# Zhouxunzhe/ManiSkill

Measured on AMD Instinct MI355X. Metric: env-steps/sec (whole node), PickCube-v1 state-obs 4096 envs/GPU, higher is better.
Workload: dtype f32; 1 GPU; PickCube-v1, Panda, state obs [N,42], pd_joint_delta_pos, num_envs=4096/GPU, sim 100 Hz / control 20 Hz = 5 substeps, 15+1 solver iterations, random actions 2*U-1, no resets inside the timed region; envs_per_gpu=4096, substeps=5, parallelism=env-sharded x1, no collective on the env path, solver_overflow_envs=0

## Files before the change

### __graft_entry__.py

```python
import os
import subprocess
import sys

ROOT = os.path.dirname(os.path.abspath(__file__))
if ROOT not in sys.path:
    sys.path.insert(0, ROOT)

HIPCC = os.environ.get("HIPCC", "/opt/rocm/bin/hipcc")
NATIVE_DIR = os.path.join(ROOT, "maniskill_amd", "_native")
SRC = os.path.join(ROOT, "maniskill_amd", "csrc", "mssim_kernels.hip")
LIB = os.path.join(NATIVE_DIR, "libmssim.so")


def _stale(target, sources):
    if not os.path.exists(target):
        return True
    t = os.path.getmtime(target)
    return any(os.path.getmtime(s) > t for s in sources)


def build(force: bool = False) -> None:
    os.makedirs(NATIVE_DIR, exist_ok=True)
    csrc = os.path.join(ROOT, "maniskill_amd", "csrc")
    deps = [os.path.join(csrc, f) for f in os.listdir(csrc)] + [os.path.join(ROOT, "include", h) for h in ("mssim.h", "mssim_hip_tasks.h")]
    if force or _stale(LIB, deps):
        tmp = f"{LIB}.{os.getpid()}.tmp"
        cmd = [HIPCC, "-O3", "--offload-arch=gfx950", "-std=c++17", "-shared", "-fPIC", "-Wno-unused-value", "-fno-hip-fp32-correctly-rounded-divide-sqrt", "-o", tmp, SRC]
        try:
            subprocess.run(cmd, check=True)
            os.replace(tmp, LIB)
        finally:
            if os.path.exists(tmp):
                os.remove(tmp)
    subprocess.run(["make", "-s", "-C", os.path.join(ROOT, "oracle")], check=True)
    import maniskill_amd
    from maniskill_amd import native

    native.NativeLib.load(LIB)


def smoke() -> None:
    import numpy as np
    import torch

    from maniskill_amd.model.scenes import panda_tabletop_model
    from maniskill_amd.physx.system import MssimSystem
    from tests import oracle_backend as ob

    assert torch.cuda.is_available(), "smoke() needs a GPU"
    build()
    model = panda_tabletop_model()
    N = 64
    g = torch.Generator().manual_seed(0)
    rest = torch.tensor([0, np.pi / 8, 0, -np.pi * 5 / 8, 0, np.pi * 3 / 4, np.pi / 4, 0.04, 0.04])
    q0 = rest + 0.02 * torch.randn(N, 9, generator=g)
    q0[:, 7:] = 0.04
    tq = q0.clone()
    tq[:, :7] += 0.1 * (2 * torch.rand(N, 7, generator=g) - 1)
    outs = []
    for dev, backend in (("cuda:0", None), ("cpu", "oracle")):
        if backend is None:
            px = MssimSystem(device=dev)
            px.gpu_init(model, N)
        else:
            px = ob.make_system(model, N, precision="f64")
        px.cuda_articulation_qpos.torch()[:] = q0.to(dev)
# ... 16 lines not shown
```

### include/mssim.h

```cpp
#ifndef MSSIM_H
#define MSSIM_H

#include <stdint.h>

#ifdef __cplusplus
extern "C" {
#endif

#define MSSIM_ABI_VERSION 6
#define MSSIM_MAX_ANGULAR_VELOCITY 100.0f
#define MSSIM_MAX_JOINT_VELOCITY 100.0f
#define MSSIM_MPR_TOLERANCE 1e-5f
#define MSSIM_PCM_SLOTS 16
#define MSSIM_PCM_DRIFT 5e-3f
#define MSSIM_PCM_MOVE 1e-3f
#define MSSIM_PCM_ROT_TRACE 2.9996f
#define MSSIM_PCM_TILT 0.05f
#define MSSIM_PCM_GROW 6
#define MSSIM_PCM_MERGE 2e-3f
#ifndef MSSIM_PGS_EXIT_TOLERANCE
#define MSSIM_PGS_EXIT_TOLERANCE 1e-6f
#endif
#define MSSIM_WAKE_TIME 0.4f
#define MSSIM_MAX_DOF 16
#define MSSIM_MAX_FREE 8
#define MSSIM_MAX_POINTS 4
#define MSSIM_MAX_HULL_VERTS 64
#define MSSIM_TRI_SLACK 4e-3f
#define MSSIM_TRI_TIE 1e-5f
#define MSSIM_MAX_TRI_HITS 32
#define MSSIM_MAX_TRI_TASKS 56
#define MSSIM_TRI_RANGE_STEPS 4
#define MSSIM_PATCH_COS 0.985f
#define MSSIM_PATCH_TIE_SEP 1e-5f
#define MSSIM_PATCH_SLACK 4e-3f
#define MSSIM_PATCH_TIE_REL 1e-3f
#define MSSIM_MAX_CONTACTS 52
#define MSSIM_MAX_HITS 64
#define MSSIM_MAX_RAW_POINTS 128

enum {
  MSSIM_OVERFLOW_HITS = 1,
  MSSIM_OVERFLOW_CONVEX = 2,
  MSSIM_OVERFLOW_RAW = 4,
  MSSIM_OVERFLOW_CONTACTS = 8,
  MSSIM_OVERFLOW_TRI = 16
};
enum { MSSIM_JOINT_REVOLUTE = 0, MSSIM_JOINT_PRISMATIC = 1 };
enum { MSSIM_DRIVE_FORCE = 0, MSSIM_DRIVE_ACCELERATION = 1 };
enum {
  MSSIM_SHAPE_PLANE = 0,
  MSSIM_SHAPE_BOX = 1,
// ... 200 lines not shown
```

### maniskill_amd/csrc/mssim_kernels.hip

```cpp
#include <hip/hip_runtime.h>

#include <cmath>
#include <cstdint>
#include <cstdio>
#include <cstdlib>
#include <cstring>
#include <algorithm>
#include <string>
#include <vector>

#include "../../include/mssim.h"
#include "../../include/mssim_hip_tasks.h"
#include "mssim_collide.h"

static_assert(sizeof(mssim_stack_task) <= sizeof(mssim_peg_task) && alignof(mssim_stack_task) <= alignof(mssim_peg_task), "tail_task union would grow");
static_assert(sizeof(mssim_pusht_task) <= sizeof(mssim_peg_task) && alignof(mssim_pusht_task) <= alignof(mssim_peg_task), "tail_task union would grow");

#define MAXC 52

struct DevModel {
  int n_dof, n_tendon, n_link, n_free, n_kin, n_shape, n_pair;
  const int *dof_parent, *dof_type, *body_gravity, *tendon_dof, *link_body, *free_gravity;
  const unsigned* dof_anc;
  const float *dof_frame, *dof_axis, *dof_limit, *dof_drive, *dof_armature, *body_inertial, *tendon_param, *link_frame;
  const float *free_inertial, *free_damping;
  const int *shape_type, *shape_kind, *shape_index, *shape_row, *shape_hull, *pair_shape;
  const int* pair_packed;
  const float *shape_frame, *shape_param, *shape_material, *shape_bound, *hull_verts;
  const float* shape_center;
  const float* dof_pack;
  const float* shape_pack;
  const float* shape_half;
  const float* tri_soup;
  const float* tri_bvh;
  const int* pair_mesh_slot;
  const int *shape_env_slot, *free_env_slot;
  const float *env_shape_frame, *env_shape_param, *env_shape_bound, *env_free_inertial;
  float gx, gy, gz, dt, contact_offset, rest_offset, erp, max_depen, sleep_threshold;
  int pos_iters, vel_iters;
};

struct DevState {
  int N;
  float *root, *q, *qd, *qt, *qdt, *qf, *qacc;
  float *free_s, *free_force, *kin;
  float* free_wake;
  float* pcm;
  int* pcm_tick;
  float* warm;
  float* tri_clear;
  float *bodypose, *bodyvel;
  float* bodyaux;
  int* pair_cnt;
  float* pair_imp;
  int* hit_list;
  float* rows;
  int* overflow;
  const float* act;
  int act_dim;
  const int* act_col;
  const float *act_lo, *act_hi;
  const int* act_flags;
  const float* act_qpos;
  float* act_target;
  float* act_target_vel;
  unsigned tail_fetch;
  mssim_buffers tail_buf;
  union { mssim_pick_task pick; mssim_push_task push; mssim_peg_task peg; mssim_stack_task stack; mssim_pusht_task pusht; } tail_task;
  const int* tail_pairs; int tail_npairs;
  float *tail_obs, *tail_reward, *tail_head;
  uint8_t* tail_flags;
};

struct TopoDyn {
  static constexpr int MAXD = MSSIM_MAX_DOF;
  static constexpr bool STATIC = false;
  static constexpr int UNROLL = 1;
  int nd;
  const int* par;
  const int* typ;
  const unsigned* ancm;
  MS_DEV TopoDyn(const DevModel& M) : nd(M.n_dof), par(M.dof_parent), typ(M.dof_type), ancm(M.dof_anc) {}
  MS_DEV int n() const { return nd; }
  MS_DEV int parent(int j) const { return par[j]; }
  MS_DEV bool revolute(int j) const { return typ[j] == MSSIM_JOINT_REVOLUTE; }
  MS_DEV unsigned anc(int j) const { return ancm[j]; }
};
struct TopoPanda {
  static constexpr int MAXD = 9;
  static constexpr bool STATIC = true;
// ... 745 lines not shown
  const int n = M.n_dof;
  const pose_t root = pose_soa(S.root, 0, N, e);
  const m3 Rr = qmat(root.q);
  const int b = M.link_body[link];
  const pose_t Pb = b < 0 ? root : pose_soa(S.bodypose, 7 * b, N, e);
  const f3 pe = pmul(Pb, pose_from(M.link_frame + 7 * link)).p;
  const unsigned path = b < 0 ? 0u : (M.dof_anc[b] | (1u << b));
  float* o = out + (size_t)e * 6 * n;
  for (int j = 0; j < n; j++) {
    f3 jv = f3{0, 0, 0}, jw = f3{0, 0, 0};
    if ((path >> j) & 1u) {
      const f3 a = f3{SOA(S.bodyaux, 6 * j), SOA(S.bodyaux, 6 * j + 1), SOA(S.bodyaux, 6 * j + 2)};
      const f3 an = f3{SOA(S.bodyaux, 6 * j + 3), SOA(S.bodyaux, 6 * j + 4), SOA(S.bodyaux, 6 * j + 5)};
      if (M.dof_type[j] == MSSIM_JOINT_REVOLUTE) { jv = cross(a, pe - an); jw = a; }
      else jv = a;
      jv = mtmulv(Rr, jv);
      jw = mtmulv(Rr, jw);
    }
    o[0 * n + j] = jv.x; o[1 * n + j] = jv.y; o[2 * n + j] = jv.z;
    o[3 * n + j] = jw.x; o[4 * n + j] = jw.y; o[5 * n + j] = jw.z;
  }
}

__global__ void k_fill(float* dst, float v, size_t count) {
  size_t i = blockIdx.x * (size_t)blockDim.x + threadIdx.x;
  if (i < count) dst[i] = v;
}
__global__ void k_i2f(const int* src, float* dst, size_t count) {
  size_t i = blockIdx.x * (size_t)blockDim.x + threadIdx.x;
  if (i < count) dst[i] = (float)src[i];
}

#include "mssim_solve16.h"

struct mssim_sim {
  int device = 0;
  int N = 0;
  DevModel M{};
  DevState S{};
  mssim_buffers buf{};
  std::vector<void*> allocs;
  std::vector<float> drive_host;
  float* d_drive = nullptr;
  bool panda = false;
  bool has_tri = false;
  int rows_per_env = 1;
  bool dirty = true;
  int n_cu = 256;
  unsigned deferred_fetch = 0u;
  const float* deferred_action = nullptr; int deferred_adim = 0, deferred_nsub = 0; hipStream_t deferred_stream = nullptr;
  std::vector<float> h_dof_pack; float* d_dof_pack = nullptr;
  std::vector<int32_t> h_shape_row, h_pair_shape;
  int* d_pick_pairs = nullptr; int n_pick_pairs = 0; int pick_rows[3] = {-1, -1, -1};
  long long n_tail_steps = 0;
  std::vector<int*> queries;
  std::vector<int> query_n;
  std::vector<int> query_kind;
  std::string err;
  int* d_act_col = nullptr; float* d_act_lo = nullptr; float* d_act_hi = nullptr; int* d_act_flags = nullptr;
  EeMap ee{-1, 0, 3, 0.f, 0.f, 0.f, 0};
  int act_max_col = -1;
  bool profiling = false;
  std::vector<hipEvent_t> ev[2];
  size_t ev_used[2] = {0, 0};
};

// ... 295 lines not shown
  {
    const bool has_es = d->n_env_shape > 0, has_ef = d->n_env_free > 0;
    if ((has_es || has_ef) && d->num_envs != num_envs) { g_create_error = "per-env arrays were built for a different num_envs"; mssim_destroy(S); return 7; }
    std::vector<int32_t> sslot(ns > 0 ? ns : 1, -1), fslot(d->n_free > 0 ? d->n_free : 1, -1);
    if (has_es) for (int i = 0; i < ns; i++) sslot[i] = d->shape_env_slot[i];
    if (has_ef) for (int i = 0; i < d->n_free; i++) fslot[i] = d->free_env_slot[i];
    if ((rc = upload(S, sslot.data(), sslot.size(), &M.shape_env_slot)) || (rc = upload(S, fslot.data(), fslot.size(), &M.free_env_slot)) ||
        (rc = upload(S, d->env_shape_frame, (size_t)7 * d->n_env_shape * num_envs, &M.env_shape_frame)) ||
        (rc = upload(S, has_es ? env_param_dev.data() : d->env_shape_param, (size_t)4 * d->n_env_shape * num_envs, &M.env_shape_param)) ||
        (rc = upload(S, d->env_shape_bound, (size_t)4 * d->n_env_shape * num_envs, &M.env_shape_bound)) ||
        (rc = upload(S, d->env_free_inertial, (size_t)10 * d->n_env_free * num_envs, &M.env_free_inertial))) {
      mssim_destroy(S);
      return rc;
    }
  }
  S->d_drive = const_cast<float*>(M.dof_drive);
  M.gx = d->gravity[0]; M.gy = d->gravity[1]; M.gz = d->gravity[2];
  M.dt = d->timestep; M.contact_offset = d->contact_offset; M.rest_offset = d->rest_offset; M.erp = d->erp;
  M.max_depen = d->max_depenetration_velocity; M.pos_iters = d->position_iterations; M.vel_iters = d->velocity_iterations;
  M.sleep_threshold = d->sleep_threshold;
  S->panda = (n == 9);
  for (int j = 0; j < n && S->panda; j++)
    if (d->dof_parent[j] != kPandaParent[j] || d->dof_type[j] != kPandaType[j]) S->panda = false;
  DevState& D = S->S;
  D.N = num_envs;
  const size_t N = (size_t)num_envs;
#define AL(field, count) if ((rc = dalloc(S, (size_t)(count) * N, &D.field))) { g_create_error = S->err; mssim_destroy(S); return rc; }
  AL(root, 7) AL(q, n) AL(qd, n) AL(qt, n) AL(qdt, n) AL(qf, n) AL(qacc, n)
  AL(free_s, 13 * d->n_free) AL(free_force, 3 * d->n_free) AL(kin, 7 * d->n_kin) AL(free_wake, d->n_free)
  AL(bodypose, 7 * n) AL(bodyvel, 6 * n) AL(bodyaux, 6 * n)
  AL(pair_cnt, d->n_pair) AL(pair_imp, 3 * d->n_pair)
  if ((rc = dalloc(S, (size_t)num_envs * S16_ROWS_GLB * S16_ROWLEN_(S->rows_per_env), &D.rows))) { g_create_error = S->err; mssim_destroy(S); return rc; }
  AL(overflow, 1)
  AL(hit_list, 1 + MAXC)
  AL(pcm_tick, 1)
  if ((rc = dalloc(S, (size_t)num_envs * MSSIM_PCM_SLOTS * S16_PCM_LEN, &D.pcm))) { g_create_error = S->err; mssim_destroy(S); return rc; }
#define HIPCHK_NEW(call) do { hipError_t _e = (call); if (_e != hipSuccess) { g_create_error = std::string(#call) + ": " + hipGetErrorString(_e); mssim_destroy(S); return 100 + (int)_e; } } while (0)
  HIPCHK_NEW(hipMemset(D.pcm, 0xFF, (size_t)num_envs * MSSIM_PCM_SLOTS * S16_PCM_LEN * sizeof(float)));
  {
    const size_t nw = (size_t)4 * (d->n_pair > 0 ? d->n_pair : 1) * N * 4;
    if ((rc = dalloc(S, nw, &D.warm))) { g_create_error = S->err; mssim_destroy(S); return rc; }
    HIPCHK_NEW(hipMemset(D.warm, 0xFF, nw * sizeof(float)));
  }
  {
    std::vector<int32_t> slot((size_t)(d->n_pair > 0 ? d->n_pair : 1), -1);
    int n_mesh_pair = 0;
    for (int p = 0; p < d->n_pair; p++)
      if (d->shape_type[d->pair_shape[2 * p + 1]] == MSSIM_SHAPE_TRIMESH) slot[p] = n_mesh_pair++;
    if ((rc = upload(S, slot.data(), slot.size(), &M.pair_mesh_slot))) { g_create_error = S->err; mssim_destroy(S); return rc; }
    std::vector<int32_t> packed((size_t)((d->n_pair + 127) / 128 * 128 + 128), -1);
    for (int p = 0; p < d->n_pair; p++) packed[p] = d->pair_shape[2 * p] | (d->pair_shape[2 * p + 1] << 8);
    if ((rc = upload(S, packed.data(), packed.size(), &M.pair_packed))) { g_create_error = S->err; mssim_destroy(S); return rc; }
    const size_t nc = (size_t)4 * (n_mesh_pair > 0 ? n_mesh_pair : 1) * N;
    if ((rc = dalloc(S, nc, &D.tri_clear))) { g_create_error = S->err; mssim_destroy(S); return rc; }
    HIPCHK_NEW(hipMemset(D.tri_clear, 0xFF, nc * sizeof(float)));
#undef HIPCHK_NEW
  }
#undef AL
  std::vector<float> ones(N, 1.0f);
  hipMemcpy(D.root + 3 * N, ones.data(), N * sizeof(float), hipMemcpyHostToDevice);
  for (int b = 0; b < d->n_free; b++) hipMemcpy(D.free_s + (13 * b + 3) * N, ones.data(), N * sizeof(float), hipMemcpyHostToDevice);
  {
    std::vector<float> awake(N * (size_t)(d->n_free > 0 ? d->n_free : 1), MSSIM_WAKE_TIME);
    if (d->n_free > 0) hipMemcpy(D.free_wake, awake.data(), awake.size() * sizeof(float), hipMemcpyHostToDevice);
  }
  for (int k = 0; k < d->n_kin; k++) hipMemcpy(D.kin + (7 * k + 3) * N, ones.data(), N * sizeof(float), hipMemcpyHostToDevice);
// ... 52 lines not shown
  return 0;
}

int mssim_fetch(mssim_handle h, uint32_t what, void* stream) {
  what |= take_deferred_fetch(h);
  flush_deferred(h, (hipStream_t)stream);
  hipLaunchKernelGGL(k_fetch, dim3(pad8((h->N + 63) / 64), h->M.n_link + h->M.n_free + h->M.n_kin + 1), dim3(64), 0, (hipStream_t)stream, h->M, h->S, h->buf, what);
  HIPCHK(h, hipGetLastError());
  return 0;
}

static void launch_fk(mssim_handle h, hipStream_t st) {
  if (h->panda) hipLaunchKernelGGL(k_fk<TopoPanda>, env_grid(h->N, 64), dim3(64), 0, st, h->M, h->S);
  else hipLaunchKernelGGL(k_fk<TopoDyn>, env_grid(h->N, 64), dim3(64), 0, st, h->M, h->S);
}

int mssim_wake_all(mssim_handle h, void* stream) {
  flush_deferred(h, (hipStream_t)stream);
  const size_t cnt = (size_t)h->M.n_free * h->N;
  if (cnt > 0) hipLaunchKernelGGL(k_fill, dim3((unsigned)((cnt + 255) / 256)), dim3(256), 0, (hipStream_t)stream, h->S.free_wake, MSSIM_WAKE_TIME, cnt);
  HIPCHK(h, hipMemsetAsync(h->S.pcm, 0xFF, (size_t)h->N * MSSIM_PCM_SLOTS * S16_PCM_LEN * sizeof(float), (hipStream_t)stream));
  HIPCHK(h, hipMemsetAsync(h->S.warm, 0xFF, (size_t)16 * (h->M.n_pair > 0 ? h->M.n_pair : 1) * h->N * sizeof(float), (hipStream_t)stream));
  HIPCHK(h, hipGetLastError());
  return 0;
}

__global__ void k_wake_envs(DevModel M, DevState S, const long long* __restrict__ idx, int n_idx) {
  const int N = S.N;
  if ((int)blockIdx.x >= n_idx) return;
  const long long e64 = idx[blockIdx.x];
  if (e64 < 0 || e64 >= N) return;
  const int e = (int)e64;
  for (int b = threadIdx.x; b < M.n_free; b += blockDim.x) SOA(S.free_wake, b) = MSSIM_WAKE_TIME;
  for (int s = threadIdx.x; s < MSSIM_PCM_SLOTS; s += blockDim.x) reinterpret_cast<int*>(S.pcm)[((size_t)e * MSSIM_PCM_SLOTS + s) * S16_PCM_LEN] = -1;
  for (int k = threadIdx.x; k < 4 * M.n_pair; k += blockDim.x) reinterpret_cast<int*>(S.warm)[((size_t)k * N + e) * 4 + 3] = -1;
}
int mssim_wake_envs(mssim_handle h, const int64_t* env_idx, int32_t n_idx, void* stream) {
  flush_deferred(h, (hipStream_t)stream);
  if (n_idx <= 0) return 0;
  if (!env_idx) { h->err = "wake_envs: no index array"; return 1; }
  hipLaunchKernelGGL(k_wake_envs, dim3((unsigned)n_idx), dim3(256), 0, (hipStream_t)stream, h->M, h->S, reinterpret_cast<const long long*>(env_idx), (int)n_idx);
  HIPCHK(h, hipGetLastError());
  return 0;
}

int mssim_update_kinematics(mssim_handle h, void* stream) {
  flush_deferred(h, (hipStream_t)stream);
  launch_fk(h, (hipStream_t)stream);
  h->dirty = false;
  HIPCHK(h, hipGetLastError());
  return 0;
}

static inline void prof_mark(mssim_handle h, int k, hipStream_t st) {
  if (!h->profiling || h->ev_used[k] >= h->ev[k].size()) return;
  (void)hipEventRecord(h->ev[k][h->ev_used[k]++], st);
}

extern "C++" {
template <int TASK>
static void launch_control_step(mssim_handle h, const DevState& S, int n_substeps, hipStream_t st);
}
int mssim_step(mssim_handle h, int32_t n_substeps, void* stream) {
  flush_deferred(h, (hipStream_t)stream);
  hipStream_t st = (hipStream_t)stream;
  if (h->dirty) { launch_fk(h, st); h->dirty = false; }
  if (n_substeps > 0) launch_control_step<0>(h, h->S, (int)n_substeps, st);
// ... 344 lines not shown

int mssim_create_pair_query(mssim_handle h, const int32_t* body_pairs, int32_t n_pairs, int32_t* qid) {
  return make_query(h, body_pairs, 2 * n_pairs, n_pairs, 0, qid);
}
int mssim_create_body_query(mssim_handle h, const int32_t* rows, int32_t n, int32_t* qid) { return make_query(h, rows, n, n, 1, qid); }

static int run_query(mssim_handle h, int32_t qid, int kind, float* out, void* stream) {
  flush_deferred(h, (hipStream_t)stream);
  if (qid < 0 || qid >= (int)h->queries.size() || h->query_kind[qid] != kind) { h->err = "bad query id"; return 1; }
  int nq = h->query_n[qid];
  if (nq == 0) return 0;
  hipLaunchKernelGGL(k_query, dim3((h->N + 255) / 256, nq), dim3(256), 0, (hipStream_t)stream, h->M, h->S, h->queries[qid], nq, kind, out);
  HIPCHK(h, hipGetLastError());
  return 0;
}
int mssim_query_pair_impulses(mssim_handle h, int32_t qid, float* out, void* stream) { return run_query(h, qid, 0, out, stream); }
int mssim_query_body_impulses(mssim_handle h, int32_t qid, float* out, void* stream) { return run_query(h, qid, 1, out, stream); }

int mssim_read_internal(mssim_handle h, const char* name, float* out, int32_t max_items, void* stream) {
  flush_deferred(h, (hipStream_t)stream);
  std::string s(name);
  const size_t N = (size_t)h->N;
  const float* src = nullptr;
  int items = 0;
  hipStream_t st = (hipStream_t)stream;
  if (s == "q") { src = h->S.q; items = h->M.n_dof; }
  else if (s == "qd") { src = h->S.qd; items = h->M.n_dof; }
  else if (s == "free") { src = h->S.free_s; items = 13 * h->M.n_free; }
  else if (s == "kin") { src = h->S.kin; items = 7 * h->M.n_kin; }
  else if (s == "free_wake") { src = h->S.free_wake; items = h->M.n_free; }
  else if (s == "root") { src = h->S.root; items = 7; }
  else if (s == "bodypose") { src = h->S.bodypose; items = 7 * h->M.n_dof; }
  else if (s == "pair_impulse") { src = h->S.pair_imp; items = 3 * h->M.n_pair; }
  else if (s == "contact_count" || s == "overflow") {
    const int* isrc = s == "overflow" ? h->S.overflow : h->S.pair_cnt;
    items = s == "overflow" ? 1 : h->M.n_pair;
    int take = items < max_items ? items : max_items;
    size_t cnt = (size_t)take * N;
    if (cnt > 0) hipLaunchKernelGGL(k_i2f, dim3((unsigned)((cnt + 255) / 256)), dim3(256), 0, st, isrc, out, cnt);
    HIPCHK(h, hipGetLastError());
    return items;
  } else {
    h->err = "unknown internal array: " + s;
    return -1;
  }
  int take = items < max_items ? items : max_items;
  if (take > 0) HIPCHK(h, hipMemcpyAsync(out, src, sizeof(float) * (size_t)take * N, hipMemcpyDeviceToDevice, st));
  return items;
}

int mssim_overflow_count(mssim_handle h, void* stream) {
  flush_deferred(h, (hipStream_t)stream);
  std::vector<int> host(h->N);
  hipStream_t st = (hipStream_t)stream;
  if (hipStreamSynchronize(st) != hipSuccess) return -1;
  if (hipMemcpy(host.data(), h->S.overflow, sizeof(int) * h->N, hipMemcpyDeviceToHost) != hipSuccess) return -1;
  (void)hipMemset(h->S.overflow, 0, sizeof(int) * h->N);
  int c = 0;
  for (int v : host) c += v != 0;
  return c;
}

}

#ifdef MSSIM_PHASE_CLOCKS
extern "C" int mssim_debug_phase_clocks(unsigned long long* out32, int reset) {
  if (hipMemcpyFromSymbol(out32, HIP_SYMBOL(g_phase_clk), 32 * sizeof(unsigned long long)) != hipSuccess) return -1;
  if (reset < 0) return 0;
  if (reset) {
// ... 25 lines not shown
```

### maniskill_amd/csrc/mssim_solve16.h

```cpp
#pragma once

#define S16_LANES 16
#ifndef S16_WAVES
#define S16_WAVES 4
#endif
#define WSYNC() do { __builtin_amdgcn_fence(__ATOMIC_RELEASE, "wavefront"); __builtin_amdgcn_wave_barrier(); __builtin_amdgcn_fence(__ATOMIC_ACQUIRE, "wavefront"); } while (0)
#define BSYNC() __syncthreads()
#ifndef S16_ENVS_PER_BLOCK
#define S16_ENVS_PER_BLOCK 4
#endif
#define S16_COM_(nr) ((nr) == 4 ? 300 : 0)
#define S16_COM S16_COM_(NR)
#define S16_ANC 8
#define S16_VEC 32
#define S16_PT 96
#define S16_PT_LINK 1
#define S16_PT_FREE 17
#define S16_MAX_FREE_(nr) ((nr) == 4 ? 6 : 2)
#define S16_MAX_FREE S16_MAX_FREE_(NR)
#define S16_PT_KIN_(nr) (S16_PT_FREE + S16_MAX_FREE_(nr))
#define S16_PT_KIN S16_PT_KIN_(NR)
#define S16_MAX_KIN 6
#define S16_MAX_SHAPE_(nr) ((nr) == 4 ? 64 : ((nr) > 1 ? 48 : 28))
#define S16_MAX_HIT 64
// ... 544 lines not shown
#pragma unroll
  for (int i = 0; i < 3; i++)
#pragma unroll
    for (int j = 0; j < 3; j++) { R[i][j] = dot(mcol(RA, i), mcol(RB, j)); AR[i][j] = fabsf(R[i][j]) + 1e-6f; }
  bool sep = false;
#pragma unroll
  for (int i = 0; i < 3; i++) sep = sep || fabsf(t[i]) > a[i] + b[0] * AR[i][0] + b[1] * AR[i][1] + b[2] * AR[i][2] + margin;
#pragma unroll
  for (int j = 0; j < 3; j++)
    sep = sep || fabsf(t[0] * R[0][j] + t[1] * R[1][j] + t[2] * R[2][j]) > b[j] + a[0] * AR[0][j] + a[1] * AR[1][j] + a[2] * AR[2][j] + margin;
#pragma unroll
  for (int i = 0; i < 3; i++)
#pragma unroll
    for (int j = 0; j < 3; j++) {
      const int i1 = (i + 1) % 3, i2 = (i + 2) % 3, j1 = (j + 1) % 3, j2 = (j + 2) % 3;
      const float ra = a[i1] * AR[i2][j] + a[i2] * AR[i1][j];
      const float rb = b[j1] * AR[i][j2] + b[j2] * AR[i][j1];
      sep = sep || fabsf(t[i2] * R[i1][j] - t[i1] * R[i2][j]) > ra + rb + margin;
    }
  return sep;
}
MS_DEV shape_t shape_from_table(const DevModel& M, const float* t) {
  shape_t sh;
  sh.c = f3{t[0], t[1], t[2]};
  sh.rot = qmat(q4{t[3], t[4], t[5], t[6]});
  sh.p0 = t[7]; sh.p1 = t[8]; sh.p2 = t[9];
  const unsigned pk = __float_as_uint(t[14]);
  sh.type = (int)(pk & 7u);
  sh.nverts = (int)((pk >> 3) & 127u);
  sh.verts = M.hull_verts + 3 * (size_t)(pk >> 15);
  return sh;
}

struct SupCoop16 {
  f3 va[4], vb[4];
  int c;
  static MS_DEV void load_one(f3 (&dst)[4], const shape_t& s, int c) {
#pragma unroll
    for (int k = 0; k < 4; k++) {
      dst[k] = f3{0, 0, 0};
      if (s.type == SH_CONVEX) {
        const int i = c + 16 * k < s.nverts ? c + 16 * k : 0;
        dst[k] = f3{s.verts[3 * i], s.verts[3 * i + 1], s.verts[3 * i + 2]};
      }
    }
  }
  static MS_DEV f3 scan(const f3 (&v)[4], const shape_t& s, f3 d, int c) {
    const f3 dl = mtmulv(s.rot, d);
    float t = dot(v[0], dl);
    int i = c;
#pragma unroll
    for (int k = 1; k < 4; k++) {
      const float tk = dot(v[k], dl);
      const bool g = tk > t && c + 16 * k < s.nverts;
      t = g ? tk : t; i = g ? c + 16 * k : i;
    }
    if (c >= s.nverts) { t = -3e38f; i = 1 << 20; }
    float tm = t;
    tm = fmaxf(tm, dpp_f<0x128>(tm)); tm = fmaxf(tm, dpp_f<0x124>(tm)); tm = fmaxf(tm, dpp_f<0x122>(tm)); tm = fmaxf(tm, dpp_f<0x121>(tm));
    int im = t == tm ? i : (1 << 20);
    im = min(im, __builtin_amdgcn_update_dpp(0, im, 0x128, 0xF, 0xF, false));
    im = min(im, __builtin_amdgcn_update_dpp(0, im, 0x124, 0xF, 0xF, false));
    im = min(im, __builtin_amdgcn_update_dpp(0, im, 0x122, 0xF, 0xF, false));
    im = min(im, __builtin_amdgcn_update_dpp(0, im, 0x121, 0xF, 0xF, false));
    const int slot = im >> 4, owner = im & 15;
    const f3 mine = sel3(slot == 0, v[0], sel3(slot == 1, v[1], sel3(slot == 2, v[2], v[3])));
    const f3 p = f3{__shfl(mine.x, owner, 16), __shfl(mine.y, owner, 16), __shfl(mine.z, owner, 16)};
    return s.c + mmulv(s.rot, p);
  }
  MS_DEV f3 operator()(int which, const shape_t& s, f3 d) const {
    if (s.type != SH_CONVEX) return support(s, d);
    if (which == 0) return scan(va, s, d, c);
    return scan(vb, s, d, c);
  }
};

template <int NDOF = 0, int TASK = 0, bool TRI = false, int NR = 1>
__global__ __launch_bounds__(64 * S16_WAVES) void k_solve16(DevModel M, DevState S, int n_sub) {
  constexpr bool FUSED = true;
  static_assert(NR == 1 || ((NR == 2 || NR == 4) && (TASK == 0 || (NR == 2 && TASK == 4))), "rows per env: 1, 2 or 4; the task tails: one row, and StackCube on two");
  constexpr int EPW = 4 / NR;
  constexpr int BLK_ENVS = S16_WAVES * EPW;
  constexpr int BLK_GRPS = S16_WAVES * 4;
  constexpr int GW = 16 * NR;
  __shared__ __attribute__((aligned(16))) float sm[BLK_ENVS * S16_ENV_FLOATS];
  __shared__ int blk_nml[BLK_ENVS];
  __shared__ int blk_nbl[BLK_ENVS];
  __shared__ int blk_ntl[BLK_ENVS];
  __shared__ int blk_npl[BLK_ENVS];
  const int N = S.N;
  const int wv = threadIdx.x >> 6, lane64 = threadIdx.x & 63;
  const int g = lane64 >> 4, c = threadIdx.x & 15;
  const int r = NR > 1 ? (g & (NR - 1)) : 0;
  const int ew = g / NR;
  const bool lead = r == 0;
  const int cl = 16 * r + c;
  const int gb = wv * EPW + ew;
  const int grp = wv * 4 + g;
  const int chunk = xcd_chunk(blockIdx.x, gridDim.x);
  if (chunk * BLK_ENVS >= N) return;
  const int e_raw = chunk * BLK_ENVS + gb;
  const bool live = e_raw < N;
  const int e = live ? e_raw : N - 1;
  float* L = sm + gb * S16_ENV_FLOATS;
  float* const smw = sm + wv * EPW * S16_ENV_FLOATS;
  const int n = NDOF > 0 ? NDOF : M.n_dof, nf = M.n_free;
  const float dt = M.dt;
  const float inv_dt = rcp_f(dt);
  const f3 g3 = f3{M.gx, M.gy, M.gz};
  const bool art = lead && c < n;
  const int fc = NR == 1 ? c - n : (r >= 1 ? c : -1);
  const bool frow = NR == 1 || r >= 1;
  const int fb0 = (NR == 4 && r >= 1) ? 2 * (r - 1) : 0;
  const int nfr = frow ? min(max(nf - fb0, 0), 2) : 0;
  const bool freel = fc >= 0 && fc < 6 * nfr;
  const int fb_id = fb0 + (freel ? fc / 6 : 0);
  const int fk = freel ? fc % 6 : 0;
  const int fcol0 = NR == 1 ? n : 0;
  const int fbase = fcol0 + 6 * (fb_id - fb0);
// ... 354 lines not shown
        }
        WSYNC();
        if (t0 == 0) {
          if (c == 0 && lead) reinterpret_cast<int*>(L)[S16_NP_ALLOC] = 0;
          WSYNC();
        }
        if (mine && m.count > 0) {
          const int off = pool_alloc(Lg, m.count);
          if (off >= 0) {
            reinterpret_cast<int*>(Lg)[S16_NP_CNT + idx] = m.count;
            reinterpret_cast<int*>(Lg)[S16_NP_OFF + idx] = off;
            float* hn = Lg + S16_NP_HN + 3 * idx;
            hn[0] = m.n.x; hn[1] = m.n.y; hn[2] = m.n.z;
#pragma unroll
            for (int k = 0; k < 4; k++)
              if (k < m.count) *reinterpret_cast<float4*>(Lg + S16_NP_POOL + 4 * (off + k)) = float4{m.x[k].x, m.x[k].y, m.x[k].z, m.sep[k]};
          }
        }
      }
      if (T == 0) {
        if (c == 0 && lead) reinterpret_cast<int*>(L)[S16_NP_ALLOC] = 0;
      }
      if (c == 0 && lead) { blk_nml[gb] = nml; blk_nbl[gb] = bb_lane ? 0 : nbl; blk_npl[gb] = npl; }
      BSYNC();
      PH(13);
      BT_T0b;
      {
        int4 hd = int4{-1, 0, 0, 0};
        if (live && nml > 0) hd = *reinterpret_cast<const int4*>(S.pcm + ((size_t)e * MSSIM_PCM_SLOTS + c) * S16_PCM_LEN);
        const int4 hd0 = hd;
        unsigned char* const slot_of = reinterpret_cast<unsigned char*>(L + S16_NP_SLOT);
        const unsigned char* const ml = reinterpret_cast<const unsigned char*>(L + S16_NP_ML);
        auto b16 = [&](bool v) __attribute__((always_inline)) { return (unsigned)(__ballot(v) >> (16 * g)) & 0xFFFFu; };
        for (int k = 0; k < nml; k++) {
          const int idx = ml[k];
          const int p = reinterpret_cast<const int*>(L)[S16_NP_HIT + idx] & 0xFFFF;
          unsigned m16 = b16(hd.x == p);
          bool fresh = false;
          if (m16 == 0u) {
            fresh = true;
            m16 = b16(hd.x < 0);
            if (m16 == 0u) {
              int st = hd.z < pcm_tick ? hd.z : 0x7FFFFFFF;
              int mn = st;
              mn = min(mn, __builtin_amdgcn_update_dpp(0, mn, 0x128, 0xF, 0xF, false));
              mn = min(mn, __builtin_amdgcn_update_dpp(0, mn, 0x124, 0xF, 0xF, false));
              mn = min(mn, __builtin_amdgcn_update_dpp(0, mn, 0x122, 0xF, 0xF, false));
              mn = min(mn, __builtin_amdgcn_update_dpp(0, mn, 0x121, 0xF, 0xF, false));
              m16 = mn != 0x7FFFFFFF ? b16(st == mn) : 0u;
            }
          }
          const int si = m16 ? (__ffs(m16) - 1) : -1;
          if (c == si) {
            if (fresh) { hd.x = p; hd.y = 0; hd.w = 0; }
            hd.z = pcm_tick;
          }
          if (c == 0) slot_of[idx] = si < 0 ? 255 : (unsigned char)(si | (fresh ? 0x80 : 0));
        }
        if (live && (hd.x != hd0.x || hd.y != hd0.y || hd.z != hd0.z || hd.w != hd0.w))
          *reinterpret_cast<int4*>(S.pcm + ((size_t)e * MSSIM_PCM_SLOTS + c) * S16_PCM_LEN) = hd;
      }
      __threadfence_block();
      BSYNC();
      BT_T(17);
      int TMb = 0;
#pragma unroll
      for (int j = 0; j < BLK_ENVS; j++) TMb += blk_nml[j];
      for (int t0 = 0; t0 < TMb; t0 += BLK_GRPS) {
        const bool has = t0 + grp < TMb;
        const int t = has ? t0 + grp : t0;
        int ge = 0, k = t;
#pragma unroll
        for (int j = 0; j < BLK_ENVS - 1; j++) {
          const int nj = blk_nml[j];
          const bool past = ge == j && k >= nj;
          k -= past ? nj : 0;
          ge += past ? 1 : 0;
        }
        float* Lg = sm + ge * S16_ENV_FLOATS;
        const int idx = reinterpret_cast<const unsigned char*>(Lg + S16_NP_ML)[k];
        const int pk = reinterpret_cast<const int*>(Lg)[S16_NP_HIT + idx];
        const shape_t A = shape_from_table(M, Lg + S16_NP_SHP + S16_SHP * ((pk >> 16) & 0xFF));
        const shape_t B = shape_from_table(M, Lg + S16_NP_SHP + S16_SHP * ((pk >> 24) & 0xFF));
        SupCoop16 sup;
        sup.c = c;
        SupCoop16::load_one(sup.va, A, c);
        SupCoop16::load_one(sup.vb, B, c);
        const int sbyte = reinterpret_cast<const unsigned char*>(Lg + S16_NP_SLOT)[idx];
        const bool cached = has && sbyte != 255;
        const bool fresh = cached && (sbyte & 0x80);
        float* const slot = S.pcm + ((size_t)(chunk * BLK_ENVS + ge) * MSSIM_PCM_SLOTS + (cached ? (sbyte & 15) : 0)) * S16_PCM_LEN;
        auto b16 = [&](bool v) __attribute__((always_inline)) { return (unsigned)(__ballot(v) >> (16 * g)) & 0xFFFFu; };
        int npts = 0, grow = 0;
        bool queried_empty = false;
        f3 relp0 = f3{0, 0, 0}, nloc = f3{1, 0, 0};
        float relR0[9] = {1, 0, 0, 0, 1, 0, 0, 0, 1};
        f3 pA = f3{0, 0, 0}, pB = f3{0, 0, 0};
        float s0 = 0.f;
        if (cached && !fresh) {
          const int4 h4 = *reinterpret_cast<const int4*>(slot);
          npts = h4.y; grow = h4.w >> 8; queried_empty = h4.w & 1;
          const float4 r1 = *reinterpret_cast<const float4*>(slot + 4), r2 = *reinterpret_cast<const float4*>(slot + 8), r3 = *reinterpret_cast<const float4*>(slot + 12),
                       r4 = *reinterpret_cast<const float4*>(slot + 16);
          relp0 = f3{r1.x, r1.y, r1.z};
          relR0[0] = r2.x; relR0[1] = r2.y; relR0[2] = r2.z; relR0[3] = r2.w; relR0[4] = r3.x; relR0[5] = r3.y; relR0[6] = r3.z; relR0[7] = r3.w; relR0[8] = r4.x;
          nloc = f3{r4.y, r4.z, r4.w};
          if (c < 4) {
            const float* pp = slot + 20 + 7 * c;
            pA = f3{pp[0], pp[1], pp[2]}; pB = f3{pp[3], pp[4], pp[5]}; s0 = pp[6];
          }
        }
        BT_T(18);
        const float offset = M.contact_offset;
        {
          const f3 nw = mmulv(A.rot, nloc);
          const f3 wA = A.c + mmulv(A.rot, pA), wB = B.c + mmulv(B.rot, pB);
          const f3 d = wA - wB;
          const float dn = dot(d, nw);
          const f3 tt = d - nw * dn;
          const bool ok = c < npts && !(dot(tt, tt) > MSSIM_PCM_DRIFT * MSSIM_PCM_DRIFT || s0 + dn > offset);
          const unsigned mk = b16(ok) & 15u;
          int src = 0;
          {
            unsigned r = mk;
            for (int q = 0; q < 4; q++) {
              const int bit = r ? (__ffs(r) - 1) : 0;
              if (q == c) src = bit;
              r &= r - 1u;
            }
          }
          pA = f3{gbc(pA.x, src), gbc(pA.y, src), gbc(pA.z, src)};
          pB = f3{gbc(pB.x, src), gbc(pB.y, src), gbc(pB.z, src)};
          s0 = gbc(s0, src);
          npts = __popc(mk);
        }
        bool moved = false;
        if (cached && !fresh) {
          const f3 dp = mtmulv(A.rot, B.c - A.c) - relp0;
          float tr = 0.f;
#pragma unroll
          for (int i = 0; i < 3; i++)
#pragma unroll
            for (int j = 0; j < 3; j++) tr += relR0[3 * i + j] * dot(mcol(A.rot, i), mcol(B.rot, j));
          moved = dot(dp, dp) > MSSIM_PCM_MOVE * MSSIM_PCM_MOVE || tr < MSSIM_PCM_ROT_TRACE;
        }
        const float relR0_8 = relR0[8];
        auto merge = [&](const m3& Rq, f3 cq, f3 gx, float gsep) __attribute__((always_inline)) {
          const f3 nA = mtmulv(Rq, gx - cq), nB = mtmulv(B.rot, gx - B.c);
          const f3 dd = nA - pA;
          const unsigned dup = b16(c < npts && dot(dd, dd) < MSSIM_PCM_MERGE * MSSIM_PCM_MERGE) & 15u;
          int at = dup ? (__ffs(dup) - 1) : (npts < 4 ? npts : 4);
          if (!dup && npts < 4) npts++;
          if (c == at) { pA = nA; pB = nB; s0 = gsep; }
          if (at < 4) return;
          const f3 nw = mmulv(A.rot, nloc);
          const f3 wA = A.c + mmulv(A.rot, pA), wB = B.c + mmulv(B.rot, pB);
          const f3 x = (wA + wB) * 0.5f;
          const float sp = s0 + dot(wA - wB, nw);
          const bool in5 = c < 5;
          float best = in5 ? sp : 3e38f;
          best = -gmax16(-best);
          const int i0 = __ffs(b16(in5 && sp <= best + MSSIM_PATCH_TIE_SEP)) - 1;
          const f3 p0 = f3{gbc(x.x, i0), gbc(x.y, i0), gbc(x.z, i0)};
          auto first_near_max = [&](float v, bool allowed, float floor_) __attribute__((always_inline)) {
            const float mx = gmax16(allowed ? v : floor_);
            if (!(mx > floor_)) return -1;
            return __ffs(b16(allowed && v >= mx - MSSIM_PATCH_TIE_REL * mx)) - 1;
          };
          const f3 d0 = x - p0;
          const int i1 = first_near_max(dot(d0, d0), in5 && c != i0, -1.f);
          const f3 ed = f3{gbc(x.x, i1), gbc(x.y, i1), gbc(x.z, i1)} - p0;
          const float ar = dot(cross(ed, x - p0), nw);
          const int i2 = first_near_max(fabsf(ar), in5 && c != i0 && c != i1, -1.f);
          const float sgn2 = gbc(ar, i2);
          const int i3 = first_near_max(sgn2 >= 0.f ? -ar : ar, in5 && c != i0 && c != i1 && c != i2, MSSIM_PATCH_TIE_REL * fabsf(sgn2));
          const unsigned keep = (1u << i0) | (1u << i1) | (1u << i2) | (i3 >= 0 ? 1u << i3 : 0u);
          int src = 0;
          {
            unsigned r = keep;
            for (int q = 0; q < 4; q++) {
              const int bit = r ? (__ffs(r) - 1) : 0;
              if (q == c) src = bit;
              r &= r - 1u;
            }
          }
          pA = f3{gbc(pA.x, src), gbc(pA.y, src), gbc(pA.z, src)};
          pB = f3{gbc(pB.x, src), gbc(pB.y, src), gbc(pB.z, src)};
          s0 = gbc(s0, src);
          npts = __popc(keep);
        };
        const bool main_q = has && (!cached || fresh || moved || (npts == 0 && !queried_empty));
        const bool growing = cached && !main_q && npts > 0 && npts < 3 && grow > 0;
        if (growing) grow--;
        BT_ADD(10, __popcll(__ballot(c == 0 && has && !cached)));
        BT_ADD(11, __popcll(__ballot(c == 0 && has && fresh)));
        BT_ADD(12, __popcll(__ballot(c == 0 && has && cached && !fresh && moved)));
        BT_ADD(13, __popcll(__ballot(c == 0 && has && cached && !fresh && !moved && main_q)));
        BT_ADD(15, __popcll(__ballot(c == 0 && has && growing)));
        BT_ADD(16, __popcll(__ballot(c == 0 && has && !main_q && !growing)));
        int mu_count = 0;
        f3 mu_n = f3{0, 0, 0}, mu_x = f3{0, 0, 0};
        float mu_sep = 0.f;
        {
          shape_t Aq = A;
          if (growing) {
            const f3 nw = mmulv(A.rot, nloc);
            const f3 wA = A.c + mmulv(A.rot, pA), wB = B.c + mmulv(B.rot, pB);
            const f3 xm = (wA + wB) * 0.5f;
            const f3 pivot = f3{gbc(xm.x, 0), gbc(xm.y, 0), gbc(xm.z, 0)};
            f3 axis;
            if (npts >= 2) axis = normalized(f3{gbc(xm.x, 1), gbc(xm.y, 1), gbc(xm.z, 1)} - pivot);
            else axis = fabsf(nw.x) < 0.57735f ? normalized(cross(nw, f3{1, 0, 0})) : normalized(cross(nw, f3{0, 1, 0}));
            if (grow & 1) axis = -axis;
            const m3 Rt = qmat(qaxis_angle(axis, MSSIM_PCM_TILT));
#pragma unroll
            for (int j = 0; j < 3; j++) {
              const f3 col = mmulv(Rt, mcol(A.rot, j));
              Aq.rot.m[0][j] = col.x; Aq.rot.m[1][j] = col.y; Aq.rot.m[2][j] = col.z;
            }
            Aq.c = pivot + mmulv(Rt, A.c - pivot);
          }
          manifold_t gq;
          manifold_clear(gq);
          BT_T(19);
          if (main_q || growing) collide_mpr_t(Aq, B, offset, gq, sup);
          BT_T(20);
          if (main_q) {
            if (!cached) {
              mu_count = gq.count; mu_n = gq.n; mu_x = gq.x[0]; mu_sep = gq.sep[0];
            } else {
              queried_empty = gq.count == 0;
              if (gq.count == 0) {
                npts = 0;
              } else {
                const f3 nnew = mtmulv(A.rot, gq.n);
                if (npts > 0 && dot(nnew, nloc) < MSSIM_PATCH_COS) npts = 0;
                if (npts == 0) grow = MSSIM_PCM_GROW;
                nloc = nnew;
                merge(A.rot, A.c, gq.x[0], gq.sep[0]);
              }
            }
          } else if (growing && gq.count > 0) {
            merge(Aq.rot, Aq.c, gq.x[0], gq.sep[0]);
          }
        }
        BT_T(21);
        if (has) {
          const f3 nw = cached ? mmulv(A.rot, nloc) : mu_n;
          const f3 wA = A.c + mmulv(A.rot, pA), wB = B.c + mmulv(B.rot, pB);
          const int cnt = cached ? npts : mu_count;
          const float4 P = cached ? float4{0.5f * (wA.x + wB.x), 0.5f * (wA.y + wB.y), 0.5f * (wA.z + wB.z), s0 + dot(wA - wB, nw)}
                                  : float4{mu_x.x, mu_x.y, mu_x.z, mu_sep};
          if (cnt > 0) {
            int off = 0;
            if (c == 0) off = pool_alloc(Lg, cnt);
            off = gbci(off, 0);
            if (off >= 0) {
              if (c == 0) {
                reinterpret_cast<int*>(Lg)[S16_NP_CNT + idx] = cnt;
                reinterpret_cast<int*>(Lg)[S16_NP_OFF + idx] = off;
                float* hn = Lg + S16_NP_HN + 3 * idx;
                hn[0] = nw.x; hn[1] = nw.y; hn[2] = nw.z;
              }
              if (c < cnt) *reinterpret_cast<float4*>(Lg + S16_NP_POOL + 4 * (off + c)) = P;
            }
          }
          if (cached) {
            if (c == 0) {
              int4 h4 = *reinterpret_cast<const int4*>(slot);
              h4.y = npts; h4.w = (grow << 8) | (queried_empty ? 1 : 0);
              *reinterpret_cast<int4*>(slot) = h4;
              float r8 = relR0_8;
              if (main_q) {
                const f3 relp = mtmulv(A.rot, B.c - A.c);
                float relR[9];
#pragma unroll
                for (int i = 0; i < 3; i++)
#pragma unroll
                  for (int j = 0; j < 3; j++) relR[3 * i + j] = dot(mcol(A.rot, i), mcol(B.rot, j));
                *reinterpret_cast<float4*>(slot + 4) = float4{relp.x, relp.y, relp.z, 0.f};
                *reinterpret_cast<float4*>(slot + 8) = float4{relR[0], relR[1], relR[2], relR[3]};
                *reinterpret_cast<float4*>(slot + 12) = float4{relR[4], relR[5], relR[6], relR[7]};
                r8 = relR[8];
              }
              *reinterpret_cast<float4*>(slot + 16) = float4{r8, nloc.x, nloc.y, nloc.z};
            }
            if (c < npts) {
              float* pp = slot + 20 + 7 * c;
              pp[0] = pA.x; pp[1] = pA.y; pp[2] = pA.z; pp[3] = pB.x; pp[4] = pB.y; pp[5] = pB.z; pp[6] = s0;
            }
          }
        }
      }
      if (TRI) {
        PH(25);
        int* const tl = reinterpret_cast<int*>(L + S16_NP_BSCR);
        int* const cand = reinterpret_cast<int*>(L + S16_NP_BSCR) + MSSIM_MAX_TRI_TASKS;
        int* const stack = reinterpret_cast<int*>(L + S16_NP_BOUT);
        int* const hitw = reinterpret_cast<int*>(L) + S16_NP_HIT;
        int* const cntw = reinterpret_cast<int*>(L) + S16_NP_CNT;
        auto b16 = [&](bool v) __attribute__((always_inline)) { return (unsigned)(__ballot(v) >> (16 * g)) & 0xFFFFu; };
        int ntask = 0;
        bool tri_over = false;
        const int nh0 = nh;
        const int* const meshl = reinterpret_cast<const int*>(L) + S16_REC;
        unsigned long long clear_mask = 0ull;
        for (int base = 0; base < nmesh; base += 16) {
          const int idx = base + c;
          bool clear_ = false;
          if (idx < nmesh) {
            const int pk = meshl[idx];
            const float* tb_ = L + S16_NP_SHP + S16_SHP * ((pk >> 24) & 0xFF);
            const int slot = M.pair_mesh_slot[pk & 0xFFFF];
            if (slot >= 0) {
              const float* ta_ = L + S16_NP_SHP + S16_SHP * ((pk >> 16) & 0xFF);
              const f3 cq = mtmulv(qmat(q4{tb_[3], tb_[4], tb_[5], tb_[6]}), f3{ta_[10], ta_[11], ta_[12]} - f3{tb_[0], tb_[1], tb_[2]});
              const float* cl = S.tri_clear + (size_t)(4 * slot) * N + e;
              const f3 dd = cq - f3{cl[0], cl[(size_t)N], cl[2 * (size_t)N]};
              const float slack = cl[3 * (size_t)N];
              clear_ = slack > 0.f && dot(dd, dd) < slack * slack;
            }
          }
// ... 1495 lines not shown
```

Baseline: 9.629 million env-steps/s.

## Skip narrowphase for cached empty pairs via separating-axis certificates

When a cached pair's MPR query returns no contact, the kernel tries to find a separating axis with a margin and stores it in the PCM slot. On later steps, pairs that moved past the PCM threshold are checked against the stored axis with one support evaluation; if separation still holds, they are removed from the narrowphase work list and the cached relative pose is refreshed, so the full MPR query is skipped. This adds a pre-pass, a compaction, and extra block syncs. It also adds a verification build variant and debug readouts (pcm_flags, cert_count).

```diff
diff --git a/__graft_entry__.py b/__graft_entry__.py
--- a/__graft_entry__.py
+++ b/__graft_entry__.py
@@ -10,6 +10,7 @@
 NATIVE_DIR = os.path.join(ROOT, "maniskill_amd", "_native")
 SRC = os.path.join(ROOT, "maniskill_amd", "csrc", "mssim_kernels.hip")
 LIB = os.path.join(NATIVE_DIR, "libmssim.so")
+LIB_CERT_VERIFY = os.path.join(NATIVE_DIR, "libmssim_certverify.so")
 
 
 def _stale(target, sources):
@@ -23,15 +24,24 @@
     os.makedirs(NATIVE_DIR, exist_ok=True)
     csrc = os.path.join(ROOT, "maniskill_amd", "csrc")
     deps = [os.path.join(csrc, f) for f in os.listdir(csrc)] + [os.path.join(ROOT, "include", h) for h in ("mssim.h", "mssim_hip_tasks.h")]
-    if force or _stale(LIB, deps):
-        tmp = f"{LIB}.{os.getpid()}.tmp"
-        cmd = [HIPCC, "-O3", "--offload-arch=gfx950", "-std=c++17", "-shared", "-fPIC", "-Wno-unused-value", "-fno-hip-fp32-correctly-rounded-divide-sqrt", "-o", tmp, SRC]
+    jobs = []
+    for target, defs in ((LIB, []), (LIB_CERT_VERIFY, ["-DEXP_CERT_VERIFY"])):
+        if force or _stale(target, deps):
+            tmp = f"{target}.{os.getpid()}.tmp"
+            cmd = [HIPCC, "-O3", "--offload-arch=gfx950", "-std=c++17", "-shared", "-fPIC", "-Wno-unused-value", "-fno-hip-fp32-correctly-rounded-divide-sqrt", *defs, "-o", tmp, SRC]
+            jobs.append((subprocess.Popen(cmd), cmd, tmp, target))
+    failed = None
+    for proc, cmd, tmp, target in jobs:
         try:
-            subprocess.run(cmd, check=True)
-            os.replace(tmp, LIB)
+            if proc.wait() == 0:
+                os.replace(tmp, target)
+            else:
+                failed = failed or subprocess.CalledProcessError(proc.returncode, cmd)
         finally:
             if os.path.exists(tmp):
                 os.remove(tmp)
+    if failed:
+        raise failed
     subprocess.run(["make", "-s", "-C", os.path.join(ROOT, "oracle")], check=True)
     import maniskill_amd
     from maniskill_amd import native
diff --git a/include/mssim.h b/include/mssim.h
--- a/include/mssim.h
+++ b/include/mssim.h
@@ -18,6 +18,7 @@
 #define MSSIM_PCM_TILT 0.05f
 #define MSSIM_PCM_GROW 6
 #define MSSIM_PCM_MERGE 2e-3f
+#define MSSIM_PCM_CERT_MARGIN (100.f * MSSIM_MPR_TOLERANCE)
 #ifndef MSSIM_PGS_EXIT_TOLERANCE
 #define MSSIM_PGS_EXIT_TOLERANCE 1e-6f
 #endif
diff --git a/maniskill_amd/csrc/mssim_kernels.hip b/maniskill_amd/csrc/mssim_kernels.hip
--- a/maniskill_amd/csrc/mssim_kernels.hip
+++ b/maniskill_amd/csrc/mssim_kernels.hip
@@ -56,6 +56,7 @@
   int* hit_list;
   float* rows;
   int* overflow;
+  int* cert_cnt;
   const float* act;
   int act_dim;
   const int* act_col;
@@ -867,6 +868,14 @@
 }
 
 #include "mssim_solve16.h"
+
+__global__ void k_pcm_flags(const float* pcm, float* dst, int N, size_t count) {
+  size_t i = blockIdx.x * (size_t)blockDim.x + threadIdx.x;
+  if (i >= count) return;
+  const size_t s = i / N, e = i % N;
+  const int* hd = reinterpret_cast<const int*>(pcm) + (e * MSSIM_PCM_SLOTS + s) * S16_PCM_LEN;
+  dst[i] = (float)hd[3];
+}
 
 struct mssim_sim {
   int device = 0;
@@ -1228,6 +1237,7 @@
   AL(pair_cnt, d->n_pair) AL(pair_imp, 3 * d->n_pair)
   if ((rc = dalloc(S, (size_t)num_envs * S16_ROWS_GLB * S16_ROWLEN_(S->rows_per_env), &D.rows))) { g_create_error = S->err; mssim_destroy(S); return rc; }
   AL(overflow, 1)
+  AL(cert_cnt, 2)
   AL(hit_list, 1 + MAXC)
   AL(pcm_tick, 1)
   if ((rc = dalloc(S, (size_t)num_envs * MSSIM_PCM_SLOTS * S16_PCM_LEN, &D.pcm))) { g_create_error = S->err; mssim_destroy(S); return rc; }
@@ -1346,7 +1356,11 @@
   if (e64 < 0 || e64 >= N) return;
   const int e = (int)e64;
   for (int b = threadIdx.x; b < M.n_free; b += blockDim.x) SOA(S.free_wake, b) = MSSIM_WAKE_TIME;
-  for (int s = threadIdx.x; s < MSSIM_PCM_SLOTS; s += blockDim.x) reinterpret_cast<int*>(S.pcm)[((size_t)e * MSSIM_PCM_SLOTS + s) * S16_PCM_LEN] = -1;
+  for (int s = threadIdx.x; s < MSSIM_PCM_SLOTS; s += blockDim.x) {
+    int* const hd = reinterpret_cast<int*>(S.pcm) + ((size_t)e * MSSIM_PCM_SLOTS + s) * S16_PCM_LEN;
+    hd[0] = -1;
+    hd[3] = 0;
+  }
   for (int k = threadIdx.x; k < 4 * M.n_pair; k += blockDim.x) reinterpret_cast<int*>(S.warm)[((size_t)k * N + e) * 4 + 3] = -1;
 }
 int mssim_wake_envs(mssim_handle h, const int64_t* env_idx, int32_t n_idx, void* stream) {
@@ -1757,9 +1771,17 @@
   else if (s == "root") { src = h->S.root; items = 7; }
   else if (s == "bodypose") { src = h->S.bodypose; items = 7 * h->M.n_dof; }
   else if (s == "pair_impulse") { src = h->S.pair_imp; items = 3 * h->M.n_pair; }
-  else if (s == "contact_count" || s == "overflow") {
-    const int* isrc = s == "overflow" ? h->S.overflow : h->S.pair_cnt;
-    items = s == "overflow" ? 1 : h->M.n_pair;
+  else if (s == "pcm_flags") {
+    items = MSSIM_PCM_SLOTS;
+    int take = items < max_items ? items : max_items;
+    size_t cnt = (size_t)take * N;
+    if (cnt > 0) hipLaunchKernelGGL(k_pcm_flags, dim3((unsigned)((cnt + 255) / 256)), dim3(256), 0, st, h->S.pcm, out, (int)N, cnt);
+    HIPCHK(h, hipGetLastError());
+    return items;
+  }
+  else if (s == "contact_count" || s == "overflow" || s == "cert_count") {
+    const int* isrc = s == "overflow" ? h->S.overflow : s == "cert_count" ? h->S.cert_cnt : h->S.pair_cnt;
+    items = s == "overflow" ? 1 : s == "cert_count" ? 2 : h->M.n_pair;
     int take = items < max_items ? items : max_items;
     size_t cnt = (size_t)take * N;
     if (cnt > 0) hipLaunchKernelGGL(k_i2f, dim3((unsigned)((cnt + 255) / 256)), dim3(256), 0, st, isrc, out, cnt);
diff --git a/maniskill_amd/csrc/mssim_solve16.h b/maniskill_amd/csrc/mssim_solve16.h
--- a/maniskill_amd/csrc/mssim_solve16.h
+++ b/maniskill_amd/csrc/mssim_solve16.h
@@ -600,6 +600,16 @@
   return sh;
 }
 
+MS_DEV bool pcm_moved(const shape_t& A, const shape_t& B, f3 relp0, const float (&relR0)[9]) {
+  const f3 dp = mtmulv(A.rot, B.c - A.c) - relp0;
+  float tr = 0.f;
+#pragma unroll
+  for (int i = 0; i < 3; i++)
+#pragma unroll
+    for (int j = 0; j < 3; j++) tr += relR0[3 * i + j] * dot(mcol(A.rot, i), mcol(B.rot, j));
+  return dot(dp, dp) > MSSIM_PCM_MOVE * MSSIM_PCM_MOVE || tr < MSSIM_PCM_ROT_TRACE;
+}
+
 struct SupCoop16 {
   f3 va[4], vb[4];
   int c;
@@ -653,6 +663,7 @@
   constexpr int GW = 16 * NR;
   __shared__ __attribute__((aligned(16))) float sm[BLK_ENVS * S16_ENV_FLOATS];
   __shared__ int blk_nml[BLK_ENVS];
+  __shared__ int blk_ncq[BLK_ENVS];
   __shared__ int blk_nbl[BLK_ENVS];
   __shared__ int blk_ntl[BLK_ENVS];
   __shared__ int blk_npl[BLK_ENVS];
@@ -1073,10 +1084,13 @@
         unsigned char* const slot_of = reinterpret_cast<unsigned char*>(L + S16_NP_SLOT);
         const unsigned char* const ml = reinterpret_cast<const unsigned char*>(L + S16_NP_ML);
         auto b16 = [&](bool v) __attribute__((always_inline)) { return (unsigned)(__ballot(v) >> (16 * g)) & 0xFFFFu; };
+        int ncq = 0;
         for (int k = 0; k < nml; k++) {
           const int idx = ml[k];
           const int p = reinterpret_cast<const int*>(L)[S16_NP_HIT + idx] & 0xFFFF;
           unsigned m16 = b16(hd.x == p);
+          const bool certq = b16(hd.x == p && hd.y == 0 && (hd.w & 3) == 3) != 0u;
+          ncq += certq ? 1 : 0;
           bool fresh = false;
           if (m16 == 0u) {
             fresh = true;
@@ -1096,14 +1110,93 @@
             if (fresh) { hd.x = p; hd.y = 0; hd.w = 0; }
             hd.z = pcm_tick;
           }
-          if (c == 0) slot_of[idx] = si < 0 ? 255 : (unsigned char)(si | (fresh ? 0x80 : 0));
-        }
+          if (c == 0) slot_of[idx] = si < 0 ? 255 : (unsigned char)(si | (fresh ? 0x80 : 0) | (certq ? 0x40 : 0));
+        }
+        if (c == 0 && lead) blk_ncq[gb] = ncq;
         if (live && (hd.x != hd0.x || hd.y != hd0.y || hd.z != hd0.z || hd.w != hd0.w))
           *reinterpret_cast<int4*>(S.pcm + ((size_t)e * MSSIM_PCM_SLOTS + c) * S16_PCM_LEN) = hd;
       }
       __threadfence_block();
       BSYNC();
       BT_T(17);
+      int NCb = 0;
+#pragma unroll
+      for (int j = 0; j < BLK_ENVS; j++) NCb += blk_ncq[j];
+      if (NCb > 0) {
+        int TM1 = 0;
+#pragma unroll
+        for (int j = 0; j < BLK_ENVS; j++) TM1 += blk_nml[j];
+        for (int t0 = 0; t0 < TM1; t0 += BLK_GRPS) {
+          const bool has = t0 + grp < TM1;
+          const int t = has ? t0 + grp : t0;
+          int ge = 0, k = t;
+#pragma unroll
+          for (int j = 0; j < BLK_ENVS - 1; j++) {
+            const int nj = blk_nml[j];
+            const bool past = ge == j && k >= nj;
+            k -= past ? nj : 0;
+            ge += past ? 1 : 0;
+          }
+          float* Lg = sm + ge * S16_ENV_FLOATS;
+          unsigned char* const mlg = reinterpret_cast<unsigned char*>(Lg + S16_NP_ML);
+          const int idx = mlg[k];
+          const int sbyte = reinterpret_cast<const unsigned char*>(Lg + S16_NP_SLOT)[idx];
+          if (has && sbyte != 255 && (sbyte & 0x40)) {
+            const int pk = reinterpret_cast<const int*>(Lg)[S16_NP_HIT + idx];
+            const shape_t A = shape_from_table(M, Lg + S16_NP_SHP + S16_SHP * ((pk >> 16) & 0xFF));
+            const shape_t B = shape_from_table(M, Lg + S16_NP_SHP + S16_SHP * ((pk >> 24) & 0xFF));
+            float* const slot = S.pcm + ((size_t)(chunk * BLK_ENVS + ge) * MSSIM_PCM_SLOTS + (sbyte & 15)) * S16_PCM_LEN;
+            const float4 r1 = *reinterpret_cast<const float4*>(slot + 4), r2 = *reinterpret_cast<const float4*>(slot + 8), r3 = *reinterpret_cast<const float4*>(slot + 12),
+                         r4 = *reinterpret_cast<const float4*>(slot + 16);
+            const float relR0[9] = {r2.x, r2.y, r2.z, r2.w, r3.x, r3.y, r3.z, r3.w, r4.x};
+            bool drop = !pcm_moved(A, B, f3{r1.x, r1.y, r1.z}, relR0);
+            if (!drop) {
+              SupCoop16 sup;
+              sup.c = c;
+              SupCoop16::load_one(sup.va, A, c);
+              SupCoop16::load_one(sup.vb, B, c);
+              const f3 nw = mmulv(A.rot, f3{r4.y, r4.z, r4.w});
+              const f3 sa = sup(0, A, nw), sb = sup(1, B, -nw);
+              if (dot(sb - sa, nw) > M.contact_offset + MSSIM_PCM_CERT_MARGIN) {
+                if (c == 0) atomicAdd(&S.cert_cnt[chunk * BLK_ENVS + ge], 1);
+#ifdef EXP_CERT_VERIFY
+                if (c == 0) reinterpret_cast<unsigned char*>(Lg + S16_NP_SLOT)[idx] = (unsigned char)(sbyte | 0x20);
+#else
+                drop = true;
+                if (c == 0) {
+                  const f3 relp = mtmulv(A.rot, B.c - A.c);
+                  float relR[9];
+#pragma unroll
+                  for (int i = 0; i < 3; i++)
+#pragma unroll
+                    for (int j = 0; j < 3; j++) relR[3 * i + j] = dot(mcol(A.rot, i), mcol(B.rot, j));
+                  *reinterpret_cast<float4*>(slot + 4) = float4{relp.x, relp.y, relp.z, 0.f};
+                  *reinterpret_cast<float4*>(slot + 8) = float4{relR[0], relR[1], relR[2], relR[3]};
+                  *reinterpret_cast<float4*>(slot + 12) = float4{relR[4], relR[5], relR[6], relR[7]};
+                  *reinterpret_cast<float4*>(slot + 16) = float4{relR[8], r4.y, r4.z, r4.w};
+                }
+#endif
+              }
+            }
+            if (drop && c == 0) mlg[k] = 255;
+          }
+        }
+        BSYNC();
+        {
+          unsigned char* const mlw = reinterpret_cast<unsigned char*>(L + S16_NP_ML);
+          auto b16 = [&](bool v) __attribute__((always_inline)) { return (unsigned)(__ballot(v) >> (16 * g)) & 0xFFFFu; };
+          int out = 0;
+          for (int b0 = 0; b0 < nml; b0 += 16) {
+            const int v = b0 + c < nml ? mlw[b0 + c] : 255;
+            const unsigned keep = b16(v != 255);
+            if (v != 255) mlw[out + __popc(keep & ((1u << c) - 1u))] = (unsigned char)v;
+            out += __popc(keep);
+          }
+          nml = out;
+          if (c == 0 && lead) blk_nml[gb] = nml;
+        }
+        BSYNC();
+      }
       int TMb = 0;
 #pragma unroll
       for (int j = 0; j < BLK_ENVS; j++) TMb += blk_nml[j];
@@ -1133,14 +1226,14 @@
         float* const slot = S.pcm + ((size_t)(chunk * BLK_ENVS + ge) * MSSIM_PCM_SLOTS + (cached ? (sbyte & 15) : 0)) * S16_PCM_LEN;
         auto b16 = [&](bool v) __attribute__((always_inline)) { return (unsigned)(__ballot(v) >> (16 * g)) & 0xFFFFu; };
         int npts = 0, grow = 0;
-        bool queried_empty = false;
+        int qflags = 0;
         f3 relp0 = f3{0, 0, 0}, nloc = f3{1, 0, 0};
         float relR0[9] = {1, 0, 0, 0, 1, 0, 0, 0, 1};
         f3 pA = f3{0, 0, 0}, pB = f3{0, 0, 0};
         float s0 = 0.f;
         if (cached && !fresh) {
           const int4 h4 = *reinterpret_cast<const int4*>(slot);
-          npts = h4.y; grow = h4.w >> 8; queried_empty = h4.w & 1;
+          npts = h4.y; grow = h4.w >> 8; qflags = h4.w & 3;
           const float4 r1 = *reinterpret_cast<const float4*>(slot + 4), r2 = *reinterpret_cast<const float4*>(slot + 8), r3 = *reinterpret_cast<const float4*>(slot + 12),
                        r4 = *reinterpret_cast<const float4*>(slot + 16);
           relp0 = f3{r1.x, r1.y, r1.z};
@@ -1176,15 +1269,7 @@
           npts = __popc(mk);
         }
         bool moved = false;
-        if (cached && !fresh) {
-          const f3 dp = mtmulv(A.rot, B.c - A.c) - relp0;
-          float tr = 0.f;
-#pragma unroll
-          for (int i = 0; i < 3; i++)
-#pragma unroll
-            for (int j = 0; j < 3; j++) tr += relR0[3 * i + j] * dot(mcol(A.rot, i), mcol(B.rot, j));
-          moved = dot(dp, dp) > MSSIM_PCM_MOVE * MSSIM_PCM_MOVE || tr < MSSIM_PCM_ROT_TRACE;
-        }
+        if (cached && !fresh) moved = pcm_moved(A, B, relp0, relR0);
         const float relR0_8 = relR0[8];
         auto merge = [&](const m3& Rq, f3 cq, f3 gx, float gsep) __attribute__((always_inline)) {
           const f3 nA = mtmulv(Rq, gx - cq), nB = mtmulv(B.rot, gx - B.c);
@@ -1230,7 +1315,7 @@
           s0 = gbc(s0, src);
           npts = __popc(keep);
         };
-        const bool main_q = has && (!cached || fresh || moved || (npts == 0 && !queried_empty));
+        const bool main_q = has && (!cached || fresh || moved || (npts == 0 && !(qflags & 1)));
         const bool growing = cached && !main_q && npts > 0 && npts < 3 && grow > 0;
         if (growing) grow--;
         BT_ADD(10, __popcll(__ballot(c == 0 && has && !cached)));
@@ -1266,11 +1351,14 @@
           BT_T(19);
           if (main_q || growing) collide_mpr_t(Aq, B, offset, gq, sup);
           BT_T(20);
+#ifdef EXP_CERT_VERIFY
+          if (c == 0 && has && cached && (sbyte & 0x20) && !(main_q && gq.count == 0)) atomicAdd(&S.cert_cnt[N + chunk * BLK_ENVS + ge], 1);
+#endif
           if (main_q) {
             if (!cached) {
               mu_count = gq.count; mu_n = gq.n; mu_x = gq.x[0]; mu_sep = gq.sep[0];
             } else {
-              queried_empty = gq.count == 0;
+              qflags = gq.count == 0 ? 1 : 0;
               if (gq.count == 0) {
                 npts = 0;
               } else {
@@ -1309,7 +1397,7 @@
           if (cached) {
             if (c == 0) {
               int4 h4 = *reinterpret_cast<const int4*>(slot);
-              h4.y = npts; h4.w = (grow << 8) | (queried_empty ? 1 : 0);
+              h4.y = npts; h4.w = (grow << 8) | qflags;
               *reinterpret_cast<int4*>(slot) = h4;
               float r8 = relR0_8;
               if (main_q) {
@@ -1329,6 +1417,24 @@
             if (c < npts) {
               float* pp = slot + 20 + 7 * c;
               pp[0] = pA.x; pp[1] = pA.y; pp[2] = pA.z; pp[3] = pB.x; pp[4] = pB.y; pp[5] = pB.z; pp[6] = s0;
+            }
+            if (main_q && qflags == 1) {
+              f3 ax = B.c - A.c;
+              bool okc = false;
+#pragma unroll 1
+              for (int tr = 0; tr < 2 && !okc; tr++) {
+                const float d2 = dot(ax, ax);
+                if (!(d2 > 1e-24f)) break;
+                ax = ax * rsq_f(d2);
+                const f3 sa = sup(0, A, ax), sb = sup(1, B, -ax);
+                okc = dot(sb - sa, ax) > offset + MSSIM_PCM_CERT_MARGIN;
+                if (!okc) ax = sb - sa;
+              }
+              if (okc && c == 0) {
+                const f3 al = mtmulv(A.rot, ax);
+                slot[17] = al.x; slot[18] = al.y; slot[19] = al.z;
+                reinterpret_cast<int*>(slot)[3] = (grow << 8) | 3;
+              }
             }
           }
         }
```

Result: no change. 9.598 million env-steps/s (-0.3%).
